# ZHANGKEON/DIS-YOLO

Measured on AMD Instinct MI355X. Metric: train images/sec @576x576 bf16, higher is better.
Workload: dtype bf16

## Files before the change

dis-yolo_amd/csrc/conv_wgrad.hip:

```cpp
#include "common.h"
#include "runtime.h"

namespace {

struct WgradParams {
  const bf16* x0;
  const bf16* x1;
  const bf16* dy;
  float* out;
  int B, H, W, C0, C1, Cin;
  int Ho, Wo, Cout, ldy;
  int ks, stride, pad_t, pad_l;
  int M, K;
  int steps_per_split, steps;
  int tilesK, tilesN;
  unsigned bytes0, bytes1, bytesy;
};

typedef __attribute__((address_space(3))) s16x4 lds_s16x4;
typedef int i32x4 __attribute__((ext_vector_type(4)));
constexpr unsigned OOB = 0x80000000u;

__device__ __forceinline__ int swz_u(int row, int u, int units) {
  const int h = (row & 3) | (((row >> 3) & 1) << 2);
  return u ^ (h & (units - 1));
}
__device__ __forceinline__ void dma16(unsigned voff, i32x4 srd, unsigned lds_dst) {
  asm volatile("s_mov_b32 m0, %2\n\ts_nop 0\n\tbuffer_load_dwordx4 %0, %1, 0 offen lds"
               :
               : "v"(voff), "s"(srd), "s"(lds_dst)
               : "memory");
}
__device__ __forceinline__ i32x4 make_srd(const void* base, unsigned bytes) {
  i32x4 r;
  r[0] = __builtin_amdgcn_readfirstlane((int)(unsigned)(size_t)base);
  r[1] = __builtin_amdgcn_readfirstlane((int)((size_t)base >> 32)) & 0xffff;
  r[2] = __builtin_amdgcn_readfirstlane((int)bytes);
  r[3] = 0x00020000;
  return r;
}
__device__ uint4 g_zero16;
__device__ __forceinline__ void dma16_flat(const void* gsrc, unsigned lds_dst) {
  asm volatile("s_mov_b32 m0, %1\n\ts_nop 0\n\tglobal_load_lds_dwordx4 %0, off" : : "v"(gsrc), "s"(lds_dst) : "memory");
}
template <int N>
__device__ __forceinline__ void wait_vmcnt() {
  asm volatile("s_waitcnt vmcnt(%0)" ::"n"(N) : "memory");
}

template <int BN, int ST>
__global__ __launch_bounds__(256) void conv_wgrad_kernel(WgradParams p) {
  constexpr int BM = 128;
  constexpr int WM = 2, WN = 2, NW = 4;
  constexpr int WTM = BM / WM, WTN = BN / WN;
  constexpr int MI = WTM / 16, NI = WTN / 16;
  constexpr int XCH = BM / 8, YCH = BN / 8;
  constexpr int XP = BM * 2, YP = BN * 2;
  constexpr int SLAB = 1024 * NW;
  constexpr int X_BYTES = 32 * XP;
  constexpr int Y_BYTES = (32 * YP + SLAB - 1) / SLAB * SLAB;
  constexpr int XI = X_BYTES / SLAB, YI = Y_BYTES / SLAB;
  constexpr int LPT = XI + YI;
  constexpr int STB = X_BYTES + Y_BYTES;
  constexpr int PRE = ST - 1;
  static_assert(WTN % 16 == 0, "BN must be a multiple of 32");

  extern __shared__ __attribute__((aligned(16))) char smem[];
  const unsigned lds0 = (unsigned)(size_t)(__attribute__((address_space(3))) char*)smem;
  const int tid = threadIdx.x, lane = tid & 63;
  const int wave = __builtin_amdgcn_readfirstlane(tid >> 6);
  const int wm = wave / WN, wn = wave % WN;
  int lin;
  {
    const int nblk = gridDim.x, bid = blockIdx.x;
    const int q = nblk >> 3, r = nblk & 7, xcd = bid & 7, loc = bid >> 3;
    lin = (xcd < r ? xcd * (q + 1) : r * (q + 1) + (xcd - r) * q) + loc;
  }
  const int bkt = lin % p.tilesK, brest = lin / p.tilesK;
  const int bnt = brest % p.tilesN, bsplit = brest / p.tilesN;
  const int kt0 = bkt * BM;
  const int n0 = bnt * BN;
  const int step0 = bsplit * p.steps_per_split;
  int step1 = step0 + p.steps_per_split;
  if (step1 > p.steps) step1 = p.steps;
  const int nsteps = step1 - step0;

  const i32x4 srd0 = make_srd(p.x0, p.bytes0);
  const i32x4 srd1 = make_srd(p.x1 ? (const void*)p.x1 : (const void*)p.x0, p.x1 ? p.bytes1 : 0u);
  const i32x4 srdy = make_srd(p.dy, p.bytesy);

  int x_kh[XI], x_kw[XI], x_ci[XI], x_b[XI], x_yo[XI], x_xo[XI];
  bool x_kok[XI], x_second[XI];
#pragma unroll
  for (int j = 0; j < XI; ++j) {
    const int chunk = (j * NW + wave) * 64 + lane;
    const int row = chunk / XCH, pc = chunk % XCH;
    const int lc = swz_u(row, pc >> 1, XCH / 2) * 2 + (pc & 1);
    const int kk = kt0 + lc * 8;
    x_kok[j] = kk < p.K;
    const int kq = x_kok[j] ? kk : 0;
    const int tap = kq / p.Cin;
    int ci = kq - tap * p.Cin;
    x_second[j] = ci >= p.C0;
    x_ci[j] = x_second[j] ? ci - p.C0 : ci;
    x_kh[j] = tap / p.ks;
    x_kw[j] = tap - x_kh[j] * p.ks;
    const int m = step0 * 32 + row;
    const int hw = p.Ho * p.Wo;
    const int b = m / hw;
    const int rem = m - b * hw;
    x_b[j] = b;
    x_yo[j] = rem / p.Wo;
    x_xo[j] = rem - x_yo[j] * p.Wo;
  }
  unsigned y_off[YI];
  int y_m[YI];
  bool y_nok[YI];
#pragma unroll
  for (int j = 0; j < YI; ++j) {
    const int chunk = (j * NW + wave) * 64 + lane;
    const int row = chunk / YCH, pc = chunk % YCH;
    const int lc = swz_u(row, pc >> 1, YCH / 2) * 2 + (pc & 1);
    const int n = n0 + lc * 8;
    y_nok[j] = (row < 32) && (n < p.ldy);
    y_m[j] = step0 * 32 + row;
    y_off[j] = ((unsigned)y_m[j] * (unsigned)p.ldy + (unsigned)n) * 2u;
  }

  const bool mixed = (p.C1 > 0) && ((p.C0 & (BM - 1)) != 0);
  const bool blk_second = (p.C1 > 0) && (kt0 >= p.C0);
  auto issue_tile = [&](int stage) {
    const unsigned sbase = lds0 + stage * STB + wave * 1024;
#pragma unroll
    for (int j = 0; j < XI; ++j) {
      const int iy = x_yo[j] * p.stride - p.pad_t + x_kh[j];
      const int ix = x_xo[j] * p.stride - p.pad_l + x_kw[j];
      const bool ok = x_kok[j] && (x_b[j] < p.B) && ((unsigned)iy < (unsigned)p.H) && ((unsigned)ix < (unsigned)p.W);
      unsigned off;
      if (!x_second[j]) {
        off = (unsigned)(((x_b[j] * p.H + iy) * p.W + ix) * p.C0 + x_ci[j]) * 2u;
      } else {
        const int H1 = p.H >> 1, W1 = p.W >> 1;
        off = (unsigned)(((x_b[j] * H1 + (iy >> 1)) * W1 + (ix >> 1)) * p.C1 + x_ci[j]) * 2u;
      }
      if (!mixed) {
        if (blk_second) dma16(ok ? off : OOB, srd1, sbase + j * SLAB);
        else dma16(ok ? off : OOB, srd0, sbase + j * SLAB);
      } else {
        const void* src = ok ? (const void*)((const char*)(x_second[j] ? p.x1 : p.x0) + off) : (const void*)&g_zero16;
        dma16_flat(src, sbase + j * SLAB);
      }
      x_xo[j] += 32;
      while (x_xo[j] >= p.Wo) {
        x_xo[j] -= p.Wo;
        if (++x_yo[j] == p.Ho) {
          x_yo[j] = 0;
          ++x_b[j];
        }
      }
    }
#pragma unroll
    for (int j = 0; j < YI; ++j) {
      dma16((y_nok[j] && y_m[j] < p.M) ? y_off[j] : OOB, srdy, sbase + X_BYTES + j * SLAB);
      y_m[j] += 32;
      y_off[j] += 32u * (unsigned)p.ldy * 2u;
    }
  };

  f32x4 acc[MI][NI];
#pragma unroll
  for (int i = 0; i < MI; ++i)
#pragma unroll
    for (int j = 0; j < NI; ++j) acc[i][j] = f32x4{0.f, 0.f, 0.f, 0.f};

#pragma unroll
  for (int s = 0; s < PRE; ++s)
    if (s < nsteps) issue_tile(s);

  const int g = lane >> 4, li = lane & 15, q = li >> 2, pc = li & 3;
  for (int st = 0; st < nsteps; ++st) {
    if (PRE >= 1 && st + PRE - 1 < nsteps)
      wait_vmcnt<LPT*(PRE >= 1 ? PRE - 1 : 0)>();
    else
      wait_vmcnt<0>();
    __builtin_amdgcn_s_barrier();
    asm volatile("" ::: "memory");
    if (st + PRE < nsteps) issue_tile((st + PRE) % ST);
    const char* sX = smem + (st % ST) * STB;
    const char* sY = sX + X_BYTES;
    bf16x8 af[MI], bfr[NI];
    typedef short s16x8 __attribute__((ext_vector_type(8)));
    const int r0 = 8 * g + q, r1 = r0 + 4;
#pragma unroll
    for (int i = 0; i < MI; ++i) {
      const int u = (wm * WTM + i * 16) >> 4;
      const s16x4 lo = __builtin_amdgcn_ds_read_tr16_b64_v4i16(
          (lds_s16x4*)(sX + r0 * XP + swz_u(r0, u, XCH / 2) * 32 + pc * 8));
      const s16x4 hi = __builtin_amdgcn_ds_read_tr16_b64_v4i16(
          (lds_s16x4*)(sX + r1 * XP + swz_u(r1, u, XCH / 2) * 32 + pc * 8));
      const s16x8 v = {lo[0], lo[1], lo[2], lo[3], hi[0], hi[1], hi[2], hi[3]};
      af[i] = __builtin_bit_cast(bf16x8, v);
    }
#pragma unroll
    for (int j = 0; j < NI; ++j) {
      const int u = (wn * WTN + j * 16) >> 4;
      const s16x4 lo = __builtin_amdgcn_ds_read_tr16_b64_v4i16(
          (lds_s16x4*)(sY + r0 * YP + swz_u(r0, u, YCH / 2) * 32 + pc * 8));
      const s16x4 hi = __builtin_amdgcn_ds_read_tr16_b64_v4i16(
          (lds_s16x4*)(sY + r1 * YP + swz_u(r1, u, YCH / 2) * 32 + pc * 8));
      const s16x8 v = {lo[0], lo[1], lo[2], lo[3], hi[0], hi[1], hi[2], hi[3]};
      bfr[j] = __builtin_bit_cast(bf16x8, v);
    }
#pragma unroll
    for (int i = 0; i < MI; ++i)
#pragma unroll
      for (int j = 0; j < NI; ++j)
        acc[i][j] = __builtin_amdgcn_mfma_f32_16x16x32_bf16(af[i], bfr[j], acc[i][j], 0, 0, 0);
  }

  float* slab = p.out + (size_t)bsplit * p.K * p.Cout;
  __syncthreads();
  constexpr int ROWP = WTN * 4 + 16;
  constexpr int HALF = MI / 2 * 16;
  if constexpr (NW * HALF * ROWP <= ST * STB) {
    if ((p.Cout & 3) == 0) {
      char* sw = smem + wave * (HALF * ROWP);
      constexpr int CPR4 = WTN / 4, CH = HALF * CPR4;
#pragma unroll
      for (int h = 0; h < 2; ++h) {
#pragma unroll
        for (int i2 = 0; i2 < MI / 2; ++i2)
#pragma unroll
          for (int j = 0; j < NI; ++j)
#pragma unroll
            for (int r = 0; r < 4; ++r)
              *reinterpret_cast<float*>(sw + (i2 * 16 + g * 4 + r) * ROWP + (j * 16 + li) * 4) = acc[h * (MI / 2) + i2][j][r];
        __builtin_amdgcn_fence(__ATOMIC_RELEASE, "wavefront");
        __builtin_amdgcn_wave_barrier();
        __builtin_amdgcn_fence(__ATOMIC_ACQUIRE, "wavefront");
#pragma unroll
        for (int it = 0; it < (CH + 63) / 64; ++it) {
          const int idx = it * 64 + lane;
          const int row = idx / CPR4, ch = idx % CPR4;
          const int kk = kt0 + wm * WTM + h * HALF + row, n = n0 + wn * WTN + ch * 4;
          if (idx < CH && kk < p.K && n < p.Cout)
            *reinterpret_cast<float4*>(slab + (size_t)kk * p.Cout + n) =
                *reinterpret_cast<const float4*>(sw + row * ROWP + ch * 16);
        }
        __builtin_amdgcn_fence(__ATOMIC_RELEASE, "wavefront");
        __builtin_amdgcn_wave_barrier();
// ... 235 lines not shown
  }

  float* slab = p.out + (size_t)bsplit * 9 * p.Cin * p.Cout;
  wait_vmcnt<0>();
  __syncthreads();
  constexpr int WTN = CO_T / 2;
  constexpr int ROWP = WTN * 4 + 16;
  constexpr int CPR4 = WTN / 4;
  char* sw = smem + wave * (16 * ROWP);
#pragma unroll
  for (int i = 0; i < TPW; ++i) {
    if (NW == 8 && i >= ntaps) continue;
    const int tap = tap0 + i;
#pragma unroll
    for (int j = 0; j < NJ; ++j)
#pragma unroll
      for (int r = 0; r < 4; ++r) *reinterpret_cast<float*>(sw + (g * 4 + r) * ROWP + (j * 16 + li) * 4) = acc[i][j][r];
    __builtin_amdgcn_fence(__ATOMIC_RELEASE, "wavefront");
    __builtin_amdgcn_wave_barrier();
    __builtin_amdgcn_fence(__ATOMIC_ACQUIRE, "wavefront");
#pragma unroll
    for (int it = 0; it < (16 * CPR4) / 64; ++it) {
      const int idx = it * 64 + lane;
      const int row = idx / CPR4, c4 = idx % CPR4;
      const int kk = tap * p.Cin + ci0 + u * 16 + row, n = co0 + ch * WTN + c4 * 4;
      if (n < p.Cout && !(p.debug & 1))
        *reinterpret_cast<float4*>(slab + (size_t)kk * p.Cout + n) = *reinterpret_cast<const float4*>(sw + row * ROWP + c4 * 16);
    }
    __builtin_amdgcn_fence(__ATOMIC_RELEASE, "wavefront");
    __builtin_amdgcn_wave_barrier();
  }
}

__global__ __launch_bounds__(256) void slab_reduce_kernel(const float* slabs, float* out, int64_t n, int splits) {
  __shared__ float sh[4][64];
  const int o = threadIdx.x & 63, g = threadIdx.x >> 6;
  const int64_t i = (int64_t)blockIdx.x * 64 + o;
  float a0 = 0.f, a1 = 0.f, a2 = 0.f, a3 = 0.f;
  if (i < n) {
    int k = g;
    for (; k + 12 < splits; k += 16) {
      a0 += slabs[(size_t)k * n + i];
      a1 += slabs[(size_t)(k + 4) * n + i];
      a2 += slabs[(size_t)(k + 8) * n + i];
      a3 += slabs[(size_t)(k + 12) * n + i];
    }
    for (; k < splits; k += 4) a0 += slabs[(size_t)k * n + i];
  }
  sh[g][o] = (a0 + a1) + (a2 + a3);
  __syncthreads();
  if (g == 0 && i < n) out[i] = (sh[0][o] + sh[1][o]) + (sh[2][o] + sh[3][o]);
}

__global__ __launch_bounds__(1024) void conv_first_wgrad_kernel(const float* img, const bf16* dy, float* slabs, int B,
                                                                int H, int W, int Cout, int px_per_block) {
  const int M = B * H * W;
  const int o = threadIdx.x;
  const int nout = 27 * Cout;
  if (o >= nout) return;
  const int k = o / Cout, co = o - k * Cout;
  const int tap = k / 3, ci = k - tap * 3;
  const int kh = tap / 3, kw = tap - kh * 3;
  const int m0 = blockIdx.x * px_per_block;
  int m1 = m0 + px_per_block;
  if (m1 > M) m1 = M;
  float acc = 0.f;
  for (int m = m0; m < m1; ++m) {
    const int b = m / (H * W);
    const int rem = m - b * H * W;
    const int y = rem / W, x = rem - y * W;
    const int iy = y + kh - 1, ix = x + kw - 1;
    if ((unsigned)iy < (unsigned)H && (unsigned)ix < (unsigned)W)
      acc += img[((size_t)(b * H + iy) * W + ix) * 3 + ci] * (float)dy[(size_t)m * Cout + co];
  }
  slabs[(size_t)blockIdx.x * nout + o] = acc;
}

constexpr int F1_ROWB = 272;
constexpr int F1_IMGB = 27 * F1_ROWB + 80;
constexpr int F1_STB = F1_IMGB + 8192;

__global__ __launch_bounds__(512) void conv_first_wgrad_mfma_kernel(const float* img, const bf16* dy, float* slabs, int B,
                                                                   int H, int W, int units_x, int nunits, unsigned bytesy) {
  extern __shared__ __attribute__((aligned(16))) char smem[];
// ... 129 lines not shown
#pragma unroll
  for (int f = 0; f < 2; ++f)
#pragma unroll
    for (int j = 0; j < 2; ++j)
#pragma unroll
      for (int r = 0; r < 4; ++r) red[((grp * 4 + wave) * 32 + 16 * f + 4 * g + r) * 32 + 16 * j + li] = acc[f][j][r];
  __syncthreads();
  float* slab = slabs + (size_t)blockIdx.x * 27 * 32;
  for (int o = threadIdx.x; o < 27 * 32; o += 512)
    slab[o] = ((red[o] + red[1024 + o]) + (red[2048 + o] + red[3072 + o])) + ((red[4096 + o] + red[5120 + o]) + (red[6144 + o] + red[7168 + o]));
}

int env_int(const char* name, int dflt) {
  const char* v = getenv(name);
  return (v && v[0]) ? atoi(v) : dflt;
}
void plan(const disyolo_conv_desc* d, int* bn, int* splits, int* steps_per_split, int* steps) {
  const int M = d->B * d->Ho * d->Wo;
  const int K = d->ksize * d->ksize * (d->C0 + d->C1);
  *bn = d->Cout > 64 ? 128 : (d->Cout > 32 ? 64 : 32);
  const int tiles = ceil_div(K, 128) * ceil_div(d->Cout, *bn);
  *steps = ceil_div(M, 32);
  static const int target = env_int("DISYOLO_WG_BLOCKS", 256);
  static const int min_steps = env_int("DISYOLO_WG_MINSTEPS", 16);
  int s = target / tiles;
  if (s < 1) s = 1;
  const int max_s = ceil_div(*steps, min_steps);
  if (s > max_s) s = max_s;
  if (s < 1) s = 1;
  *steps_per_split = ceil_div(*steps, s);
  *splits = ceil_div(*steps, *steps_per_split);
}


struct Plan3 {
  int co_t, R, splits, cps, chunks, tilesCi, tilesCo, leadA, leadB, st, s2;
  size_t lds;
};
bool plan3(const disyolo_conv_desc* d, int opts, Plan3* q) {
  static const int enabled = env_int("DISYOLO_WG3", 1);
  static const int s2_enabled = env_int("DISYOLO_WG3_S2", 1);
  static const int target = env_int("DISYOLO_WG3_BLOCKS", 192);
  if (!enabled || (opts & DISYOLO_WGRAD_IM2COL)) return false;
  if (d->ksize != 3 || d->C1 != 0 || d->in_div != 1 || d->C0 % 32 || d->Cout % 4 || d->Cout < 32) return false;
  q->s2 = 0;
  if (d->stride == 2) {
    if (!s2_enabled || d->pad_t != 0 || d->pad_l != 0 || (d->H & 1) || (d->W & 1) || d->Ho * 2 != d->H || d->Wo * 2 != d->W) return false;
    q->s2 = 1;
  } else if (d->stride != 1 || d->pad_t != 1 || d->pad_l != 1 || d->Ho != d->H || d->Wo != d->W) {
    return false;
  }
  const int P = d->Wo + 1, Hp = d->Ho + 1;
  static const int cot_env = env_int("DISYOLO_WG3_COT", 0);
  q->co_t = d->Cout > 64 ? 128 : 64;
  if (cot_env == 64) q->co_t = 64;
  if (cot_env == 0 && q->co_t == 128) {
    const int t128 = (d->C0 / 32) * ceil_div(d->Cout, 128);
    if ((target + t128 / 2) / t128 == 2) q->co_t = 64;
  }
  q->leadB = q->s2 ? 0 : ceil_div(P + 1, 64);
  q->leadA = 1 + P / 64;
  if (q->s2) q->co_t = 64;
  static const int st_env = env_int("DISYOLO_WG3_ST", 3);
  q->st = st_env < 3 ? 3 : (st_env > 5 ? 5 : st_env);
  for (;;) {
    const int need = (q->st - 1) + q->leadA + q->leadB + 1;
// ... 101 lines not shown
    Wg3Params p;
    p.x = (const bf16*)d->x0;
    p.dy = (const bf16*)dy;
    p.B = d->B; p.H = d->H; p.W = d->W; p.Cin = d->C0; p.Cout = d->Cout; p.ldy = dy_ld;
    p.Ho = d->Ho; p.Wo = d->Wo;
    p.P = d->Wo + 1; p.Hp = d->Ho + 1; p.frame = p.Hp * p.P;
    p.kbias = q3.s2 ? 0 : ceil_div((q3.leadB + 1) * 64, p.frame);
    p.a64 = 64 / p.P; p.r64 = 64 % p.P;
    p.chunks = q3.chunks; p.chunks_per_split = q3.cps;
    p.tilesCi = q3.tilesCi; p.tilesCo = q3.tilesCo; p.tiles = q3.tilesCi * q3.tilesCo;
    p.leadA = q3.leadA; p.leadB = q3.leadB;
    p.bytesx = (unsigned)((size_t)d->B * d->H * d->W * d->C0 * 2);
    p.bytesy = (unsigned)((size_t)d->B * d->Ho * d->Wo * dy_ld * 2);
    p.out = q3.splits == 1 ? dw : (float*)workspace;
    static const int dbg = env_int("DISYOLO_WG3_DEBUG", 0);
    p.debug = dbg;
    hipStream_t s = (hipStream_t)stream;
    if (opts & DISYOLO_WGRAD_REDUCE_ONLY) goto reduce3;
    if (q3.s2) {
      launch3_s2(p, q3, s);
    } else if (q3.co_t == 128) {
      if (q3.R == 8) launch3<128, 8>(p, q3, s);
      else if (q3.R == 16) launch3<128, 16>(p, q3, s);
      else launch3<128, 32>(p, q3, s);
    } else {
      if (q3.R == 8) launch3<64, 8>(p, q3, s);
      else if (q3.R == 16) launch3<64, 16>(p, q3, s);
      else launch3<64, 32>(p, q3, s);
    }
    DY_CHECK_LAUNCH();
  reduce3:
    if (q3.splits > 1 && !(opts & DISYOLO_WGRAD_PARTIAL_ONLY)) {
      const int64_t n = (int64_t)9 * p.Cin * p.Cout;
      hipLaunchKernelGGL(slab_reduce_kernel, dim3(ceil_div(n, 64)), dim3(256), 0, s, (const float*)workspace, dw, n,
                         q3.splits);
      DY_CHECK_LAUNCH();
    }
    return DISYOLO_OK;
  }
  WgradParams p;
  p.x0 = (const bf16*)d->x0;
  p.x1 = (const bf16*)d->x1;
  p.dy = (const bf16*)dy;
  p.B = d->B; p.H = d->H; p.W = d->W; p.C0 = d->C0; p.C1 = d->C1; p.Cin = d->C0 + d->C1;
  p.Ho = d->Ho; p.Wo = d->Wo; p.Cout = d->Cout; p.ldy = dy_ld;
  p.ks = d->ksize; p.stride = d->stride; p.pad_t = d->pad_t; p.pad_l = d->pad_l;
  p.M = d->B * d->Ho * d->Wo;
  p.K = d->ksize * d->ksize * p.Cin;
  p.bytes0 = (unsigned)((size_t)d->B * d->H * d->W * d->C0 * 2);
  p.bytes1 = (unsigned)((size_t)d->B * (d->H / 2) * (d->W / 2) * d->C1 * 2);
  p.bytesy = (unsigned)((size_t)p.M * dy_ld * 2);
  int bn, splits;
  plan(d, &bn, &splits, &p.steps_per_split, &p.steps);
  p.out = splits == 1 ? dw : (float*)workspace;
  hipStream_t s = (hipStream_t)stream;
  p.tilesK = ceil_div(p.K, 128);
  p.tilesN = ceil_div(p.Cout, bn);
  dim3 grid(p.tilesK * p.tilesN * splits);
  const int sto = (opts & DISYOLO_WGRAD_STAGES_MASK) >> 4;
  const int st = sto ? sto + 1 : 3;
  if (opts & DISYOLO_WGRAD_REDUCE_ONLY) goto reduce1;
#define DY_WG(BNV, YB)                                                                                   \
  if (st == 2) hipLaunchKernelGGL((conv_wgrad_kernel<BNV, 2>), grid, dim3(256), 2 * (8192 + YB), s, p);      \
  else if (st == 3) hipLaunchKernelGGL((conv_wgrad_kernel<BNV, 3>), grid, dim3(256), 3 * (8192 + YB), s, p); \
  else hipLaunchKernelGGL((conv_wgrad_kernel<BNV, 4>), grid, dim3(256), 4 * (8192 + YB), s, p);
  if (bn == 128) { DY_WG(128, 8192) }
  else if (bn == 64) { DY_WG(64, 4096) }
  else { DY_WG(32, 4096) }
#undef DY_WG
  DY_CHECK_LAUNCH();
reduce1:
  if (splits > 1 && !(opts & DISYOLO_WGRAD_PARTIAL_ONLY)) {
    const int64_t n = (int64_t)p.K * p.Cout;
    hipLaunchKernelGGL(slab_reduce_kernel, dim3(ceil_div(n, 64)), dim3(256), 0, s, (const float*)workspace, dw, n,
                       splits);
    DY_CHECK_LAUNCH();
  }
  return DISYOLO_OK;
}

static int first_wgrad_blocks(int B, int H, int W) {
  const int64_t pairs = ((int64_t)B * H * ceil_div(W, 128) + 1) / 2;
  return (int)(pairs < 512 ? pairs : 512);
}

extern "C" size_t disyolo_conv_first_wgrad_workspace(int B, int H, int W, int Cout) {
  const int64_t M = (int64_t)B * H * W;
  const int blocks = ceil_div(M, 1024);
  const size_t direct = (size_t)blocks * 27 * Cout * sizeof(float);
  const size_t mfma = (size_t)first_wgrad_blocks(B, H, W) * 27 * 32 * sizeof(float);
  return direct > mfma ? direct : mfma;
}

extern "C" int disyolo_conv_first_wgrad(const float* images, const void* dy, float* dw, int B, int H, int W, int Cout,
                                        void* workspace, size_t workspace_bytes, void* stream) {
  DY_REQUIRE(images && dy && dw && B > 0 && H > 0 && W > 0 && Cout > 0 && 27 * Cout <= 1024, "first_wgrad: bad args");
  if (!workspace || workspace_bytes < disyolo_conv_first_wgrad_workspace(B, H, W, Cout)) {
    disyolo_set_error("first_wgrad: workspace too small");
    return DISYOLO_E_WORKSPACE;
  }
  DY_RECORD_OR_RUN([=](void* s) { return disyolo_conv_first_wgrad(images, dy, dw, B, H, W, Cout, workspace, workspace_bytes, s); });
  const int64_t M = (int64_t)B * H * W;
  hipStream_t s = (hipStream_t)stream;
  const int64_t n = 27 * Cout;
  static const int use_mfma = env_int("DISYOLO_FIRST_WGRAD_MFMA", 1);
  if (Cout == 32 && use_mfma && M * 64 < (1LL << 31)) {
    const int units_x = ceil_div(W, 128);
    const int nunits = B * H * units_x;
    const int blocks = first_wgrad_blocks(B, H, W);
    hipLaunchKernelGGL(conv_first_wgrad_mfma_kernel, dim3(blocks), dim3(512), 4 * F1_STB, s, images, (const bf16*)dy,
                       (float*)workspace, B, H, W, units_x, nunits, (unsigned)(M * 64));
    DY_CHECK_LAUNCH();
    hipLaunchKernelGGL(slab_reduce_kernel, dim3(ceil_div(n, 64)), dim3(256), 0, s, (const float*)workspace, dw, n, blocks);
    DY_CHECK_LAUNCH();
    return DISYOLO_OK;
  }
  const int blocks = ceil_div(M, 1024);
  hipLaunchKernelGGL(conv_first_wgrad_kernel, dim3(blocks), dim3(1024), 0, s, images, (const bf16*)dy,
                     (float*)workspace, B, H, W, Cout, 1024);
  DY_CHECK_LAUNCH();
  hipLaunchKernelGGL(slab_reduce_kernel, dim3(ceil_div(n, 64)), dim3(256), 0, s, (const float*)workspace, dw, n,
                     blocks);
  DY_CHECK_LAUNCH();
  return DISYOLO_OK;
}
```

dis-yolo_amd/csrc/ops.hip:

```cpp
#include <stdarg.h>
#include <stdlib.h>
#include "common.h"
#include "runtime.h"

static thread_local char g_err[512] = "";
void disyolo_set_error(const char* fmt, ...) {
  va_list ap;
  va_start(ap, fmt);
  vsnprintf(g_err, sizeof(g_err), fmt, ap);
  va_end(ap);
}
extern "C" const char* disyolo_last_error(void) { return g_err; }
extern "C" int disyolo_version(void) { return 100; }

namespace {

template <int COUT, bool FP8OUT = false>
__global__ __launch_bounds__(256) void conv_first_kernel(const float* __restrict__ img, const float* __restrict__ sw,
                                                         const float* __restrict__ ssc,
                                                         const float* __restrict__ ssh, bf16* __restrict__ y, int B,
                                                         int H, int W, float alpha, float inv_out_scale = 0.f) {
  __shared__ uint4 stage[4][64 * (COUT / 8)];
  const int lane = threadIdx.x & 63, wave = threadIdx.x >> 6;
  const int64_t total = (int64_t)B * H * W;
// ... 207 lines not shown
  for (int i = threadIdx.x; i < 64 * 64; i += 256) {
    const int kk = i / 64, nn = i % 64;
    float v = 0.f;
    if (k0 + kk < K && n0 + nn < Cout) v = w[(size_t)(k0 + kk) * Cout + n0 + nn];
    t[kk][nn] = v;
  }
  __syncthreads();
  for (int i = threadIdx.x; i < 64 * 64; i += 256) {
    const int nn = i / 64, kk = i % 64;
    if (k0 + kk < K && n0 + nn < Cout) out[(size_t)(n0 + nn) * K + k0 + kk] = (bf16)t[kk][nn];
  }
}
__global__ __launch_bounds__(256) void pack_dgrad_kernel(const float* w, bf16* out, int taps, int Cin, int Cout,
                                                         int cout_pad) {
  const int64_t total = (int64_t)Cin * taps * cout_pad;
  const int64_t stride = (int64_t)gridDim.x * blockDim.x;
  for (int64_t i = (int64_t)blockIdx.x * blockDim.x + threadIdx.x; i < total; i += stride) {
    const int co = (int)(i % cout_pad);
    const int64_t r = i / cout_pad;
    const int tp = (int)(r % taps);
    const int ci = (int)(r / taps);
    float v = 0.f;
    if (co < Cout) v = w[((size_t)(taps - 1 - tp) * Cin + ci) * Cout + co];
    out[i] = (bf16)v;
  }
}

struct PackJob {
  const float* w;
  bf16* fwd;
  bf16* dgrad;
  int K, Cout, Cin, taps, cout_pad;
  int blk0;
  int blk1;
  int tiles_k;
};
__global__ __launch_bounds__(256) void pack_all_kernel(const PackJob* jobs, int njobs) {
  __shared__ float t[64][65];
  int lo = 0, hi = njobs - 1;
  const int bid = blockIdx.x;
  while (lo < hi) {
    const int mid = (lo + hi + 1) >> 1;
    if (jobs[mid].blk0 <= bid) lo = mid; else hi = mid - 1;
  }
  const PackJob j = jobs[lo];
  if (bid < j.blk1) {
    const int tb = bid - j.blk0;
    const int k0 = (tb % j.tiles_k) * 64, n0 = (tb / j.tiles_k) * 64;
    for (int i = threadIdx.x; i < 64 * 64; i += 256) {
      const int kk = i / 64, nn = i % 64;
      float v = 0.f;
      if (k0 + kk < j.K && n0 + nn < j.Cout) v = j.w[(size_t)(k0 + kk) * j.Cout + n0 + nn];
      t[kk][nn] = v;
    }
    __syncthreads();
    for (int i = threadIdx.x; i < 64 * 64; i += 256) {
      const int nn = i / 64, kk = i % 64;
      if (k0 + kk < j.K && n0 + nn < j.Cout) j.fwd[(size_t)(n0 + nn) * j.K + k0 + kk] = (bf16)t[kk][nn];
    }
  } else {
    const int64_t total = (int64_t)j.Cin * j.taps * j.cout_pad;
    const int64_t base = (int64_t)(bid - j.blk1) * 4096;
    for (int e = threadIdx.x; e < 4096; e += 256) {
      const int64_t i = base + e;
      if (i >= total) break;
      const int co = (int)(i % j.cout_pad);
      const int64_t r = i / j.cout_pad;
      const int tp = (int)(r % j.taps);
      const int ci = (int)(r / j.taps);
      float v = 0.f;
      if (co < j.Cout) v = j.w[((size_t)(j.taps - 1 - tp) * j.Cin + ci) * j.Cout + co];
      j.dgrad[i] = (bf16)v;
    }
  }
}

__global__ __launch_bounds__(256) void adam_kernel(float* w, const float* g, float* m, float* v, int64_t n,
                                                   int64_t n_decay, float lr_t, float b1, float b2, float eps,
                                                   float l2, float gscale) {
  const int64_t stride = (int64_t)gridDim.x * blockDim.x;
  for (int64_t i = (int64_t)blockIdx.x * blockDim.x + threadIdx.x; i < n; i += stride) {
    const float wi = w[i];
    float gi = g[i] * gscale;
    if (i < n_decay) gi += l2 * wi;
    const float mi = b1 * m[i] + (1.f - b1) * gi;
    const float vi = b2 * v[i] + (1.f - b2) * gi * gi;
    m[i] = mi;
    v[i] = vi;
    w[i] = wi - lr_t * mi / (sqrtf(vi) + eps);
  }
}

__global__ __launch_bounds__(256) void adam_dev_kernel(float* w, const float* g, float* m, float* v, int64_t n,
                                                       int64_t n_decay, float lr, float b1, float b2, float eps,
                                                       float l2, float gscale, const int64_t* counter) {
  const double t = (double)(*counter + 1);
  const float lr_t = (float)((double)lr * sqrt(1.0 - pow((double)b2, t)) / (1.0 - pow((double)b1, t)));
  const int64_t stride = (int64_t)gridDim.x * blockDim.x;
  for (int64_t i = (int64_t)blockIdx.x * blockDim.x + threadIdx.x; i < n; i += stride) {
    const float wi = w[i];
    float gi = g[i] * gscale;
    if (i < n_decay) gi += l2 * wi;
    const float mi = b1 * m[i] + (1.f - b1) * gi;
    const float vi = b2 * v[i] + (1.f - b2) * gi * gi;
    m[i] = mi;
// ... 170 lines not shown
  DY_RECORD_OR_RUN([=](void* s) { return disyolo_pack_weights(w_hwio, w_fwd, w_dgrad, ksize, Cin, Cout, cout_pad, s); });
  hipStream_t s = (hipStream_t)stream;
  const int taps = ksize * ksize, K = taps * Cin;
  if (w_fwd) {
    hipLaunchKernelGGL(pack_fwd_kernel, dim3(ceil_div(K, 64), ceil_div(Cout, 64)), dim3(256), 0, s, w_hwio,
                       (bf16*)w_fwd, K, Cout);
    DY_CHECK_LAUNCH();
  }
  if (w_dgrad) {
    const int64_t total = (int64_t)Cin * taps * cout_pad;
    int grid = ceil_div(total, 256);
    if (grid > 4096) grid = 4096;
    hipLaunchKernelGGL(pack_dgrad_kernel, dim3(grid), dim3(256), 0, s, w_hwio, (bf16*)w_dgrad, taps, Cin, Cout,
                       cout_pad);
    DY_CHECK_LAUNCH();
  }
  return DISYOLO_OK;
}

extern "C" size_t disyolo_pack_table_bytes(int njobs) { return (size_t)njobs * sizeof(PackJob); }

extern "C" int disyolo_pack_table_build(const disyolo_pack_job* jobs, int njobs, void* host_table, int* total_blocks) {
  DY_REQUIRE(jobs && njobs > 0 && host_table && total_blocks, "pack_table_build: bad args");
  PackJob* t = (PackJob*)host_table;
  int blk = 0;
  for (int i = 0; i < njobs; ++i) {
    const disyolo_pack_job& s = jobs[i];
    DY_REQUIRE(s.w_hwio && s.w_fwd && s.ksize > 0 && s.Cin > 0 && s.Cout > 0, "pack_table_build: job %d incomplete", i);
    PackJob& d = t[i];
    d.w = s.w_hwio; d.fwd = (bf16*)s.w_fwd; d.dgrad = (bf16*)s.w_dgrad;
    d.taps = s.ksize * s.ksize; d.K = d.taps * s.Cin; d.Cout = s.Cout; d.Cin = s.Cin;
    d.cout_pad = s.cout_pad > s.Cout ? s.cout_pad : s.Cout;
    d.tiles_k = ceil_div(d.K, 64);
    d.blk0 = blk;
    blk += d.tiles_k * ceil_div(d.Cout, 64);
    d.blk1 = blk;
    if (d.dgrad) blk += ceil_div((int64_t)d.Cin * d.taps * d.cout_pad, 4096);
  }
  *total_blocks = blk;
  return DISYOLO_OK;
}

extern "C" int disyolo_pack_all(const void* device_table, int njobs, int total_blocks, void* stream) {
  DY_REQUIRE(device_table && njobs > 0 && total_blocks > 0, "pack_all: bad args");
  DY_RECORD_OR_RUN([=](void* s) { return disyolo_pack_all(device_table, njobs, total_blocks, s); });
  hipLaunchKernelGGL(pack_all_kernel, dim3(total_blocks), dim3(256), 0, (hipStream_t)stream, (const PackJob*)device_table,
                     njobs);
  DY_CHECK_LAUNCH();
  return DISYOLO_OK;
}

extern "C" int disyolo_adam_step(float* w, const float* grad, float* m, float* v, int64_t n, int64_t n_decay, float lr,
                                 float beta1, float beta2, float eps, float l2, int64_t t, float grad_scale,
                                 void* stream) {
  DY_REQUIRE(w && grad && m && v && n > 0 && t >= 1 && n_decay >= 0 && n_decay <= n, "adam: bad args");
  DY_RECORD_OR_RUN([=](void* s) { return disyolo_adam_step(w, grad, m, v, n, n_decay, lr, beta1, beta2, eps, l2, t, grad_scale, s); });
  const double lr_t = (double)lr * sqrt(1.0 - pow((double)beta2, (double)t)) / (1.0 - pow((double)beta1, (double)t));
  int grid = ceil_div(n, 256);
  if (grid > 256 * 16) grid = 256 * 16;
  hipLaunchKernelGGL(adam_kernel, dim3(grid), dim3(256), 0, (hipStream_t)stream, w, grad, m, v, n, n_decay,
                     (float)lr_t, beta1, beta2, eps, l2, grad_scale);
  DY_CHECK_LAUNCH();
  return DISYOLO_OK;
}

extern "C" int disyolo_adam_step_dev(float* w, const float* grad, float* m, float* v, int64_t n, int64_t n_decay,
                                     float lr, float beta1, float beta2, float eps, float l2, int64_t* step_counter,
                                     float grad_scale, void* stream) {
  DY_REQUIRE(w && grad && m && v && step_counter && n > 0 && n_decay >= 0 && n_decay <= n, "adam_dev: bad args");
  DY_RECORD_OR_RUN([=](void* s) {
// ... 100 lines not shown
```

Measured before the change: 2184.

## Add BM/pixel-per-stage wgrad variants and vectorized multi-chunk slab reduction

The wgrad kernel now takes BM and PS (pixel-steps per pipeline stage) as template parameters, and small-K, narrow-N convolutions use a BM=64, PS=2, 4-stage variant so each DMA stage carries more pixels per barrier. The slab reduction kernel is rewritten to load float4 vectors, unroll deeper across splits, and, when there are many splits, divide them among thread groups inside the block. Launching goes through a helper that raises the dynamic LDS limit when needed. The aim is fewer barriers and better tile use for small layers and a cheaper split-K reduction, at the cost of more LDS and more template instantiations.

```diff
diff --git a/dis-yolo_amd/csrc/conv_wgrad.hip b/dis-yolo_amd/csrc/conv_wgrad.hip
--- a/dis-yolo_amd/csrc/conv_wgrad.hip
+++ b/dis-yolo_amd/csrc/conv_wgrad.hip
@@ -48,22 +48,24 @@
   asm volatile("s_waitcnt vmcnt(%0)" ::"n"(N) : "memory");
 }
 
-template <int BN, int ST>
+template <int BM, int BN, int PS, int ST>
 __global__ __launch_bounds__(256) void conv_wgrad_kernel(WgradParams p) {
-  constexpr int BM = 128;
   constexpr int WM = 2, WN = 2, NW = 4;
   constexpr int WTM = BM / WM, WTN = BN / WN;
   constexpr int MI = WTM / 16, NI = WTN / 16;
   constexpr int XCH = BM / 8, YCH = BN / 8;
   constexpr int XP = BM * 2, YP = BN * 2;
   constexpr int SLAB = 1024 * NW;
-  constexpr int X_BYTES = 32 * XP;
-  constexpr int Y_BYTES = (32 * YP + SLAB - 1) / SLAB * SLAB;
+  constexpr int PX = 32 * PS;
+  constexpr int X_BYTES = PX * XP;
+  constexpr int Y_BYTES = (PX * YP + SLAB - 1) / SLAB * SLAB;
   constexpr int XI = X_BYTES / SLAB, YI = Y_BYTES / SLAB;
   constexpr int LPT = XI + YI;
   constexpr int STB = X_BYTES + Y_BYTES;
   constexpr int PRE = ST - 1;
-  static_assert(WTN % 16 == 0, "BN must be a multiple of 32");
+  static_assert(WTN % 16 == 0 && WTM % 32 == 0, "BN must be a multiple of 32, BM of 64");
+  static_assert(X_BYTES % SLAB == 0, "the input image of a stage is a whole number of block-wide DMAs");
+  static_assert(LPT * PRE < 64, "vmcnt counts to 63");
 
   extern __shared__ __attribute__((aligned(16))) char smem[];
   const unsigned lds0 = (unsigned)(size_t)(__attribute__((address_space(3))) char*)smem;
@@ -84,12 +86,14 @@
   int step1 = step0 + p.steps_per_split;
   if (step1 > p.steps) step1 = p.steps;
   const int nsteps = step1 - step0;
+  const int nst = (nsteps + PS - 1) / PS;
+  const int mend = step1 * 32 < p.M ? step1 * 32 : p.M;
 
   const i32x4 srd0 = make_srd(p.x0, p.bytes0);
   const i32x4 srd1 = make_srd(p.x1 ? (const void*)p.x1 : (const void*)p.x0, p.x1 ? p.bytes1 : 0u);
   const i32x4 srdy = make_srd(p.dy, p.bytesy);
 
-  int x_kh[XI], x_kw[XI], x_ci[XI], x_b[XI], x_yo[XI], x_xo[XI];
+  int x_kh[XI], x_kw[XI], x_ci[XI], x_b[XI], x_yo[XI], x_xo[XI], x_m[XI];
   bool x_kok[XI], x_second[XI];
 #pragma unroll
   for (int j = 0; j < XI; ++j) {
@@ -106,6 +110,7 @@
     x_kh[j] = tap / p.ks;
     x_kw[j] = tap - x_kh[j] * p.ks;
     const int m = step0 * 32 + row;
+    x_m[j] = m;
     const int hw = p.Ho * p.Wo;
     const int b = m / hw;
     const int rem = m - b * hw;
@@ -122,7 +127,7 @@
     const int row = chunk / YCH, pc = chunk % YCH;
     const int lc = swz_u(row, pc >> 1, YCH / 2) * 2 + (pc & 1);
     const int n = n0 + lc * 8;
-    y_nok[j] = (row < 32) && (n < p.ldy);
+    y_nok[j] = (row < PX) && (n < p.ldy);
     y_m[j] = step0 * 32 + row;
     y_off[j] = ((unsigned)y_m[j] * (unsigned)p.ldy + (unsigned)n) * 2u;
   }
@@ -135,7 +140,7 @@
     for (int j = 0; j < XI; ++j) {
       const int iy = x_yo[j] * p.stride - p.pad_t + x_kh[j];
       const int ix = x_xo[j] * p.stride - p.pad_l + x_kw[j];
-      const bool ok = x_kok[j] && (x_b[j] < p.B) && ((unsigned)iy < (unsigned)p.H) && ((unsigned)ix < (unsigned)p.W);
+      const bool ok = x_kok[j] && (x_m[j] < mend) && ((unsigned)iy < (unsigned)p.H) && ((unsigned)ix < (unsigned)p.W);
       unsigned off;
       if (!x_second[j]) {
         off = (unsigned)(((x_b[j] * p.H + iy) * p.W + ix) * p.C0 + x_ci[j]) * 2u;
@@ -150,7 +155,8 @@
         const void* src = ok ? (const void*)((const char*)(x_second[j] ? p.x1 : p.x0) + off) : (const void*)&g_zero16;
         dma16_flat(src, sbase + j * SLAB);
       }
-      x_xo[j] += 32;
+      x_m[j] += PX;
+      x_xo[j] += PX;
       while (x_xo[j] >= p.Wo) {
         x_xo[j] -= p.Wo;
         if (++x_yo[j] == p.Ho) {
@@ -161,9 +167,9 @@
     }
 #pragma unroll
     for (int j = 0; j < YI; ++j) {
-      dma16((y_nok[j] && y_m[j] < p.M) ? y_off[j] : OOB, srdy, sbase + X_BYTES + j * SLAB);
-      y_m[j] += 32;
-      y_off[j] += 32u * (unsigned)p.ldy * 2u;
+      dma16((y_nok[j] && y_m[j] < mend) ? y_off[j] : OOB, srdy, sbase + X_BYTES + j * SLAB);
+      y_m[j] += PX;
+      y_off[j] += (unsigned)PX * (unsigned)p.ldy * 2u;
     }
   };
 
@@ -175,22 +181,26 @@
 
 #pragma unroll
   for (int s = 0; s < PRE; ++s)
-    if (s < nsteps) issue_tile(s);
+    if (s < nst) issue_tile(s);
 
   const int g = lane >> 4, li = lane & 15, q = li >> 2, pc = li & 3;
-  for (int st = 0; st < nsteps; ++st) {
-    if (PRE >= 1 && st + PRE - 1 < nsteps)
+  for (int st = 0; st < nst; ++st) {
+    if (PRE >= 1 && st + PRE - 1 < nst)
       wait_vmcnt<LPT*(PRE >= 1 ? PRE - 1 : 0)>();
     else
       wait_vmcnt<0>();
     __builtin_amdgcn_s_barrier();
     asm volatile("" ::: "memory");
-    if (st + PRE < nsteps) issue_tile((st + PRE) % ST);
+    if (st + PRE < nst) issue_tile((st + PRE) % ST);
+    const int nsub = nsteps - st * PS;
+#pragma unroll
+    for (int sub = 0; sub < PS; ++sub) {
+    if (sub >= nsub) break;
     const char* sX = smem + (st % ST) * STB;
     const char* sY = sX + X_BYTES;
     bf16x8 af[MI], bfr[NI];
     typedef short s16x8 __attribute__((ext_vector_type(8)));
-    const int r0 = 8 * g + q, r1 = r0 + 4;
+    const int r0 = sub * 32 + 8 * g + q, r1 = r0 + 4;
 #pragma unroll
     for (int i = 0; i < MI; ++i) {
       const int u = (wm * WTM + i * 16) >> 4;
@@ -216,6 +226,7 @@
 #pragma unroll
       for (int j = 0; j < NI; ++j)
         acc[i][j] = __builtin_amdgcn_mfma_f32_16x16x32_bf16(af[i], bfr[j], acc[i][j], 0, 0, 0);
+    }
   }
 
   float* slab = p.out + (size_t)bsplit * p.K * p.Cout;
@@ -517,24 +528,106 @@
   }
 }
 
+struct f4 {
+  float v[4];
+};
+__device__ __forceinline__ f4 slab_load4(const float* s, int64_t i, int64_t n, bool vec) {
+  f4 r;
+  if (vec) {
+    const float4 t = *reinterpret_cast<const float4*>(s + i);
+    r.v[0] = t.x; r.v[1] = t.y; r.v[2] = t.z; r.v[3] = t.w;
+  } else {
+#pragma unroll
+    for (int e = 0; e < 4; ++e) r.v[e] = i + e < n ? s[i + e] : 0.f;
+  }
+  return r;
+}
+template <int CH>
 __global__ __launch_bounds__(256) void slab_reduce_kernel(const float* slabs, float* out, int64_t n, int splits) {
-  __shared__ float sh[4][64];
-  const int o = threadIdx.x & 63, g = threadIdx.x >> 6;
-  const int64_t i = (int64_t)blockIdx.x * 64 + o;
-  float a0 = 0.f, a1 = 0.f, a2 = 0.f, a3 = 0.f;
+  constexpr int Q = 64 / CH;
+  __shared__ float sh[4][CH][Q][4];
+  const int o = threadIdx.x % Q, c = (threadIdx.x / Q) % CH, g = threadIdx.x / (Q * CH);
+  const int64_t i = ((int64_t)blockIdx.x * Q + o) * 4;
+  const bool vec = (n & 3) == 0;
+  float a[4][4];
+#pragma unroll
+  for (int j = 0; j < 4; ++j)
+#pragma unroll
+    for (int e = 0; e < 4; ++e) a[j][e] = 0.f;
   if (i < n) {
+    const float* s = slabs;
+    const size_t sn = (size_t)n;
     int k = g;
-    for (; k + 12 < splits; k += 16) {
-      a0 += slabs[(size_t)k * n + i];
-      a1 += slabs[(size_t)(k + 4) * n + i];
-      a2 += slabs[(size_t)(k + 8) * n + i];
-      a3 += slabs[(size_t)(k + 12) * n + i];
-    }
-    for (; k < splits; k += 4) a0 += slabs[(size_t)k * n + i];
-  }
-  sh[g][o] = (a0 + a1) + (a2 + a3);
+    if constexpr (CH == 1) {
+      for (; k + 28 < splits; k += 32) {
+        f4 v[8];
+#pragma unroll
+        for (int j = 0; j < 8; ++j) v[j] = slab_load4(s + (size_t)(k + 4 * j) * sn, i, n, vec);
+#pragma unroll
+        for (int j = 0; j < 8; ++j)
+#pragma unroll
+          for (int e = 0; e < 4; ++e) a[j & 3][e] += v[j].v[e];
+      }
+      for (; k + 12 < splits; k += 16) {
+        f4 v[4];
+#pragma unroll
+        for (int j = 0; j < 4; ++j) v[j] = slab_load4(s + (size_t)(k + 4 * j) * sn, i, n, vec);
+#pragma unroll
+        for (int j = 0; j < 4; ++j)
+#pragma unroll
+          for (int e = 0; e < 4; ++e) a[j][e] += v[j].v[e];
+      }
+    } else {
+      int t = 0;
+      for (; k + 16 * (t + 3) + 12 < splits; t += 4) {
+        f4 v[4];
+#pragma unroll
+        for (int u = 0; u < 4; ++u) v[u] = slab_load4(s + (size_t)(k + 4 * c + 16 * (t + u)) * sn, i, n, vec);
+#pragma unroll
+        for (int u = 0; u < 4; ++u)
+#pragma unroll
+          for (int e = 0; e < 4; ++e) a[0][e] += v[u].v[e];
+      }
+      for (; k + 16 * t + 12 < splits; ++t) {
+        const f4 v = slab_load4(s + (size_t)(k + 4 * c + 16 * t) * sn, i, n, vec);
+#pragma unroll
+        for (int e = 0; e < 4; ++e) a[0][e] += v.v[e];
+      }
+      k += 16 * t;
+    }
+    if (CH == 1 || c == 0) {
+      for (; k < splits; k += 4) {
+        const f4 v = slab_load4(s + (size_t)k * sn, i, n, vec);
+#pragma unroll
+        for (int e = 0; e < 4; ++e) a[0][e] += v.v[e];
+      }
+    }
+  }
+  if constexpr (CH == 1) {
+#pragma unroll
+    for (int e = 0; e < 4; ++e) sh[g][0][o][e] = (a[0][e] + a[1][e]) + (a[2][e] + a[3][e]);
+  } else {
+#pragma unroll
+    for (int e = 0; e < 4; ++e) sh[g][c][o][e] = a[0][e];
+  }
   __syncthreads();
-  if (g == 0 && i < n) out[i] = (sh[0][o] + sh[1][o]) + (sh[2][o] + sh[3][o]);
+  if (threadIdx.x < Q * 4) {
+    const int oo = threadIdx.x >> 2, e = threadIdx.x & 3;
+    const int64_t io = ((int64_t)blockIdx.x * Q + oo) * 4 + e;
+    float sg[4];
+#pragma unroll
+    for (int gg = 0; gg < 4; ++gg) {
+      if constexpr (CH == 1) sg[gg] = sh[gg][0][oo][e];
+      else sg[gg] = (sh[gg][0][oo][e] + sh[gg][1][oo][e]) + (sh[gg][2][oo][e] + sh[gg][3][oo][e]);
+    }
+    if (io < n) out[io] = (sg[0] + sg[1]) + (sg[2] + sg[3]);
+  }
+}
+void launch_slab_reduce(const float* slabs, float* out, int64_t n, int splits, hipStream_t s) {
+  if (splits > 32)
+    hipLaunchKernelGGL(slab_reduce_kernel<4>, dim3(ceil_div(n, 64)), dim3(256), 0, s, slabs, out, n, splits);
+  else
+    hipLaunchKernelGGL(slab_reduce_kernel<1>, dim3(ceil_div(n, 256)), dim3(256), 0, s, slabs, out, n, splits);
 }
 
 __global__ __launch_bounds__(1024) void conv_first_wgrad_kernel(const float* img, const bf16* dy, float* slabs, int B,
@@ -730,6 +823,22 @@
   *splits = ceil_div(*steps, *steps_per_split);
 }
 
+
+template <int BM, int BN, int PS, int ST>
+void launch1(const WgradParams& p, dim3 grid, hipStream_t s) {
+  constexpr int YB = (32 * PS * BN * 2 + 4095) / 4096 * 4096;
+  constexpr int LDS = ST * (32 * PS * BM * 2 + YB);
+  static_assert(LDS <= 160 * 1024, "LDS of one CU");
+  auto fn = conv_wgrad_kernel<BM, BN, PS, ST>;
+  if constexpr (LDS > 64 * 1024) {
+    static bool attr_done = false;
+    if (!attr_done) {
+      if (hipFuncSetAttribute((const void*)fn, hipFuncAttributeMaxDynamicSharedMemorySize, LDS) != hipSuccess) (void)hipGetLastError();
+      attr_done = true;
+    }
+  }
+  hipLaunchKernelGGL(fn, grid, dim3(256), LDS, s, p);
+}
 
 struct Plan3 {
   int co_t, R, splits, cps, chunks, tilesCi, tilesCo, leadA, leadB, st, s2;
@@ -897,8 +1006,7 @@
   reduce3:
     if (q3.splits > 1 && !(opts & DISYOLO_WGRAD_PARTIAL_ONLY)) {
       const int64_t n = (int64_t)9 * p.Cin * p.Cout;
-      hipLaunchKernelGGL(slab_reduce_kernel, dim3(ceil_div(n, 64)), dim3(256), 0, s, (const float*)workspace, dw, n,
-                         q3.splits);
+      launch_slab_reduce((const float*)workspace, dw, n, q3.splits, s);
       DY_CHECK_LAUNCH();
     }
     return DISYOLO_OK;
@@ -919,26 +1027,36 @@
   plan(d, &bn, &splits, &p.steps_per_split, &p.steps);
   p.out = splits == 1 ? dw : (float*)workspace;
   hipStream_t s = (hipStream_t)stream;
-  p.tilesK = ceil_div(p.K, 128);
+  const int sto = (opts & DISYOLO_WGRAD_STAGES_MASK) >> 4;
+  const int st = sto + 1;
+  const int bm = (!sto && bn == 32 && p.K <= 64) ? 64 : 128;
+  p.tilesK = ceil_div(p.K, bm);
   p.tilesN = ceil_div(p.Cout, bn);
   dim3 grid(p.tilesK * p.tilesN * splits);
-  const int sto = (opts & DISYOLO_WGRAD_STAGES_MASK) >> 4;
-  const int st = sto ? sto + 1 : 3;
   if (opts & DISYOLO_WGRAD_REDUCE_ONLY) goto reduce1;
-#define DY_WG(BNV, YB)                                                                                   \
-  if (st == 2) hipLaunchKernelGGL((conv_wgrad_kernel<BNV, 2>), grid, dim3(256), 2 * (8192 + YB), s, p);      \
-  else if (st == 3) hipLaunchKernelGGL((conv_wgrad_kernel<BNV, 3>), grid, dim3(256), 3 * (8192 + YB), s, p); \
-  else hipLaunchKernelGGL((conv_wgrad_kernel<BNV, 4>), grid, dim3(256), 4 * (8192 + YB), s, p);
-  if (bn == 128) { DY_WG(128, 8192) }
-  else if (bn == 64) { DY_WG(64, 4096) }
-  else { DY_WG(32, 4096) }
+  if (sto) {
+#define DY_WG(BNV)                                                   \
+  if (st == 2) launch1<128, BNV, 1, 2>(p, grid, s);                  \
+  else if (st == 3) launch1<128, BNV, 1, 3>(p, grid, s);             \
+  else launch1<128, BNV, 1, 4>(p, grid, s);
+    if (bn == 128) { DY_WG(128) }
+    else if (bn == 64) { DY_WG(64) }
+    else { DY_WG(32) }
 #undef DY_WG
+  } else if (bn == 128) {
+    launch1<128, 128, 1, 3>(p, grid, s);
+  } else if (bn == 64) {
+    launch1<128, 64, 1, 3>(p, grid, s);
+  } else if (bm == 64) {
+    launch1<64, 32, 2, 4>(p, grid, s);
+  } else {
+    launch1<128, 32, 1, 3>(p, grid, s);
+  }
   DY_CHECK_LAUNCH();
 reduce1:
   if (splits > 1 && !(opts & DISYOLO_WGRAD_PARTIAL_ONLY)) {
     const int64_t n = (int64_t)p.K * p.Cout;
-    hipLaunchKernelGGL(slab_reduce_kernel, dim3(ceil_div(n, 64)), dim3(256), 0, s, (const float*)workspace, dw, n,
-                       splits);
+    launch_slab_reduce((const float*)workspace, dw, n, splits, s);
     DY_CHECK_LAUNCH();
   }
   return DISYOLO_OK;
@@ -976,7 +1094,7 @@
     hipLaunchKernelGGL(conv_first_wgrad_mfma_kernel, dim3(blocks), dim3(512), 4 * F1_STB, s, images, (const bf16*)dy,
                        (float*)workspace, B, H, W, units_x, nunits, (unsigned)(M * 64));
     DY_CHECK_LAUNCH();
-    hipLaunchKernelGGL(slab_reduce_kernel, dim3(ceil_div(n, 64)), dim3(256), 0, s, (const float*)workspace, dw, n, blocks);
+    launch_slab_reduce((const float*)workspace, dw, n, blocks, s);
     DY_CHECK_LAUNCH();
     return DISYOLO_OK;
   }
@@ -984,8 +1102,7 @@
   hipLaunchKernelGGL(conv_first_wgrad_kernel, dim3(blocks), dim3(1024), 0, s, images, (const bf16*)dy,
                      (float*)workspace, B, H, W, Cout, 1024);
   DY_CHECK_LAUNCH();
-  hipLaunchKernelGGL(slab_reduce_kernel, dim3(ceil_div(n, 64)), dim3(256), 0, s, (const float*)workspace, dw, n,
-                     blocks);
+  launch_slab_reduce((const float*)workspace, dw, n, blocks, s);
   DY_CHECK_LAUNCH();
   return DISYOLO_OK;
 }
```

Result: no change. 2180, median of 2 (-0.2%).

## Fuse forward and dgrad weight packing into one vectorized tiled pass

Applied to the files above, without the earlier changes.

Reworks the weight pack kernel so each 64x64 tile reads the HWIO fp32 weights once and writes both the transposed forward layout and the flipped dgrad layout. Loads use float4 and stores use 16-byte writes when alignment allows, and the LDS transpose uses an XOR swizzle on packed bf16 pairs. This removes the separate dgrad pass with its per-element div/mod and strided reads. The cost is a more complex kernel with alignment-dependent paths and more blocks when cout_pad exceeds Cout.

```diff
diff --git a/dis-yolo_amd/csrc/ops.hip b/dis-yolo_amd/csrc/ops.hip
--- a/dis-yolo_amd/csrc/ops.hip
+++ b/dis-yolo_amd/csrc/ops.hip
@@ -263,11 +263,11 @@
   bf16* dgrad;
   int K, Cout, Cin, taps, cout_pad;
   int blk0;
-  int blk1;
   int tiles_k;
+  int vec;
 };
 __global__ __launch_bounds__(256) void pack_all_kernel(const PackJob* jobs, int njobs) {
-  __shared__ float t[64][65];
+  __shared__ __attribute__((aligned(16))) uint2 t[64 * 16];
   int lo = 0, hi = njobs - 1;
   const int bid = blockIdx.x;
   while (lo < hi) {
@@ -275,33 +275,89 @@
     if (jobs[mid].blk0 <= bid) lo = mid; else hi = mid - 1;
   }
   const PackJob j = jobs[lo];
-  if (bid < j.blk1) {
-    const int tb = bid - j.blk0;
-    const int k0 = (tb % j.tiles_k) * 64, n0 = (tb / j.tiles_k) * 64;
-    for (int i = threadIdx.x; i < 64 * 64; i += 256) {
-      const int kk = i / 64, nn = i % 64;
-      float v = 0.f;
-      if (k0 + kk < j.K && n0 + nn < j.Cout) v = j.w[(size_t)(k0 + kk) * j.Cout + n0 + nn];
-      t[kk][nn] = v;
-    }
-    __syncthreads();
-    for (int i = threadIdx.x; i < 64 * 64; i += 256) {
-      const int nn = i / 64, kk = i % 64;
-      if (k0 + kk < j.K && n0 + nn < j.Cout) j.fwd[(size_t)(n0 + nn) * j.K + k0 + kk] = (bf16)t[kk][nn];
-    }
-  } else {
-    const int64_t total = (int64_t)j.Cin * j.taps * j.cout_pad;
-    const int64_t base = (int64_t)(bid - j.blk1) * 4096;
-    for (int e = threadIdx.x; e < 4096; e += 256) {
-      const int64_t i = base + e;
-      if (i >= total) break;
-      const int co = (int)(i % j.cout_pad);
-      const int64_t r = i / j.cout_pad;
-      const int tp = (int)(r % j.taps);
-      const int ci = (int)(r / j.taps);
-      float v = 0.f;
-      if (co < j.Cout) v = j.w[((size_t)(j.taps - 1 - tp) * j.Cin + ci) * j.Cout + co];
-      j.dgrad[i] = (bf16)v;
+  const int tb = bid - j.blk0;
+  const int k0 = (tb % j.tiles_k) * 64, n0 = (tb / j.tiles_k) * 64;
+  const int c4 = threadIdx.x & 15, r = threadIdx.x >> 4;
+  const int co = n0 + 4 * c4, kq = k0 + 4 * r;
+  float4 x[4];
+#pragma unroll
+  for (int p = 0; p < 4; ++p) {
+    float4 v = {0.f, 0.f, 0.f, 0.f};
+    if (kq + p < j.K) {
+      const float* src = j.w + (size_t)(kq + p) * j.Cout + co;
+      if (j.vec & 1) {
+        if (co < j.Cout) v = *reinterpret_cast<const float4*>(src);
+      } else {
+        if (co < j.Cout) v.x = src[0];
+        if (co + 1 < j.Cout) v.y = src[1];
+        if (co + 2 < j.Cout) v.z = src[2];
+        if (co + 3 < j.Cout) v.w = src[3];
+      }
+    }
+    x[p] = v;
+  }
+  if (j.dgrad) {
+    unsigned a[4], b[4];
+    size_t row[4];
+    int tap = k0 / j.Cin, ci = kq - tap * j.Cin;
+#pragma unroll
+    for (int p = 0; p < 4; ++p) {
+      while (ci >= j.Cin) { ci -= j.Cin; ++tap; }
+      row[p] = (size_t)ci * j.taps + (j.taps - 1 - tap);
+      ++ci;
+      a[p] = pack2(x[p].x, x[p].y);
+      b[p] = pack2(x[p].z, x[p].w);
+    }
+    if (j.vec & 4) {
+      const bool odd = c4 & 1;
+      const int col = n0 + 8 * (c4 >> 1);
+#pragma unroll
+      for (int q = 0; q < 2; ++q) {
+        const unsigned ga = __shfl_xor(odd ? a[q] : a[2 + q], 1, 64), gb = __shfl_xor(odd ? b[q] : b[2 + q], 1, 64);
+        const unsigned ma = odd ? a[2 + q] : a[q], mb = odd ? b[2 + q] : b[q];
+        const uint4 o = odd ? make_uint4(ga, gb, ma, mb) : make_uint4(ma, mb, ga, gb);
+        const int k = kq + q + (odd ? 2 : 0);
+        const size_t rw = odd ? row[2 + q] : row[q];
+        if (k < j.K && col < j.cout_pad) *reinterpret_cast<uint4*>(j.dgrad + rw * j.cout_pad + col) = o;
+      }
+    } else {
+      unsigned short* dg = reinterpret_cast<unsigned short*>(j.dgrad);
+#pragma unroll
+      for (int p = 0; p < 4; ++p) {
+        if (kq + p >= j.K) continue;
+        unsigned short* dst = dg + row[p] * j.cout_pad + co;
+        if (co < j.cout_pad) dst[0] = (unsigned short)a[p];
+        if (co + 1 < j.cout_pad) dst[1] = (unsigned short)(a[p] >> 16);
+        if (co + 2 < j.cout_pad) dst[2] = (unsigned short)b[p];
+        if (co + 3 < j.cout_pad) dst[3] = (unsigned short)(b[p] >> 16);
+      }
+    }
+  }
+  if (n0 >= j.Cout) return;
+  t[(4 * c4 + 0) * 16 + (r ^ c4)] = make_uint2(pack2(x[0].x, x[1].x), pack2(x[2].x, x[3].x));
+  t[(4 * c4 + 1) * 16 + (r ^ c4)] = make_uint2(pack2(x[0].y, x[1].y), pack2(x[2].y, x[3].y));
+  t[(4 * c4 + 2) * 16 + (r ^ c4)] = make_uint2(pack2(x[0].z, x[1].z), pack2(x[2].z, x[3].z));
+  t[(4 * c4 + 3) * 16 + (r ^ c4)] = make_uint2(pack2(x[0].w, x[1].w), pack2(x[2].w, x[3].w));
+  __syncthreads();
+#pragma unroll
+  for (int pass = 0; pass < 2; ++pass) {
+    const int cl = (threadIdx.x >> 3) + 32 * pass, jj = threadIdx.x & 7;
+    const int f = (cl >> 2) & 15;
+    uint4 u = *reinterpret_cast<const uint4*>(&t[cl * 16 + 2 * (jj ^ (f >> 1))]);
+    if (f & 1) u = make_uint4(u.z, u.w, u.x, u.y);
+    const int k = k0 + 8 * jj;
+    if (n0 + cl >= j.Cout) continue;
+    bf16* dst = j.fwd + (size_t)(n0 + cl) * j.K + k;
+    if (j.vec & 2) {
+      if (k < j.K) *reinterpret_cast<uint4*>(dst) = u;
+    } else {
+      unsigned short* d = reinterpret_cast<unsigned short*>(dst);
+      const unsigned e[4] = {u.x, u.y, u.z, u.w};
+#pragma unroll
+      for (int i = 0; i < 4; ++i) {
+        if (k + 2 * i < j.K) d[2 * i] = (unsigned short)e[i];
+        if (k + 2 * i + 1 < j.K) d[2 * i + 1] = (unsigned short)(e[i] >> 16);
+      }
     }
   }
 }
@@ -538,10 +594,10 @@
     d.taps = s.ksize * s.ksize; d.K = d.taps * s.Cin; d.Cout = s.Cout; d.Cin = s.Cin;
     d.cout_pad = s.cout_pad > s.Cout ? s.cout_pad : s.Cout;
     d.tiles_k = ceil_div(d.K, 64);
+    d.vec = (d.Cout % 4 == 0 && ((size_t)d.w & 15) == 0 ? 1 : 0) | (d.K % 8 == 0 && ((size_t)d.fwd & 15) == 0 ? 2 : 0) |
+            (d.dgrad && d.cout_pad % 8 == 0 && ((size_t)d.dgrad & 15) == 0 ? 4 : 0);
     d.blk0 = blk;
-    blk += d.tiles_k * ceil_div(d.Cout, 64);
-    d.blk1 = blk;
-    if (d.dgrad) blk += ceil_div((int64_t)d.Cin * d.taps * d.cout_pad, 4096);
+    blk += d.tiles_k * ceil_div(d.dgrad ? d.cout_pad : d.Cout, 64);
   }
   *total_blocks = blk;
   return DISYOLO_OK;
```

New measurement: 2164 before, 2163 after. No clear change (-0.0%).
